# jyf588/SimGAN

Measured on AMD Instinct MI355X. Metric: env-steps/sec of GAIL-dyn PPO update, higher is better.
Workload: dtype f32; 1 GPU; northstar: GAIL-dyn update, T=128 N=512/GPU obs=47 act=12 D-in=86 policy=mlp h64 D h100 ppo_epoch=10 num_mini_batch=1...; optimizer_steps_per_update=2720, parallelism=single GPU

## Files before the change

simgan_amd/csrc/sg_disc_step4.hpp:

```cpp
#pragma once

struct Step4Args {
    PregatherArgs next;
    double* loss_acc;
};

#define SG_STEP4_TIMEOUT_TICKS 300000000ll

__device__ __forceinline__ float sg_ld_sc1(__amdgpu_buffer_rsrc_t r, int byte_off) {
    return __uint_as_float(__builtin_amdgcn_raw_buffer_load_b32(r, byte_off, 0, 16 ));
}

__device__ __forceinline__ bool sg_step4_wait(const unsigned* flags, int lo, int hi, unsigned want, int lane) {
    const long long deadline = wall_clock64() + SG_STEP4_TIMEOUT_TICKS;
    for (int it = 0;; ++it) {
        bool ok = true;
        for (int j = lo + lane; j < hi; j += 64) ok = ok & (__hip_atomic_load(flags + j * SG_STEP4_FLAG_STRIDE, __ATOMIC_RELAXED, __HIP_MEMORY_SCOPE_AGENT) == want);
        if (__all(ok)) return true;
        if ((it & 31) == 31 && wall_clock64() > deadline) return false;
        __builtin_amdgcn_s_sleep(1);
    }
}

#define SG_STEP4_POLLS 1
#define SG_STEP4_POLL_START_TICKS 340
struct SgStep4Polls { unsigned r[SG_STEP4_POLLS] = {}; };
__device__ __forceinline__ unsigned sg_step4_poll(const unsigned* p) {
    unsigned r;
    asm volatile("global_load_dword %0, %1, off sc1" : "=v"(r) : "v"(p) : "memory");
    return r;
}
__device__ __forceinline__ bool sg_step4_wait_piped(SgStep4Polls& pp, const unsigned* flags, int n, unsigned want, int lane, const int* quit) {
    constexpr int K = SG_STEP4_POLLS;
    static_assert(K >= 1 && K <= 3, "SG_STEP4_POLLS: 1, 2 or 3");
    const unsigned* p = flags + (lane < n ? lane : n - 1) * SG_STEP4_FLAG_STRIDE;
    const long long deadline = wall_clock64() + SG_STEP4_TIMEOUT_TICKS;
#pragma unroll
    for (int i = 0; i < K; ++i) {
        pp.r[i] = sg_step4_poll(p);
        if (i + 1 < K) __builtin_amdgcn_s_sleep(28 / K);
    }
    for (int it = 0;; ++it) {
#pragma unroll
        for (int i = 0; i < K; ++i) {
            asm volatile("s_waitcnt vmcnt(%1)" : "+v"(pp.r[i]) : "n"(K - 1) : "memory");
            if (__all(pp.r[i] == want)) return true;
            __builtin_amdgcn_s_sleep(1);
            pp.r[i] = sg_step4_poll(p);
        }
        if ((it & 31) == 31 && (wall_clock64() > deadline || __hip_atomic_load(quit, __ATOMIC_RELAXED, __HIP_MEMORY_SCOPE_WORKGROUP) == 2)) return false;
    }
}
__device__ __forceinline__ void sg_step4_polls_retire(SgStep4Polls& pp) {
#pragma unroll
    for (int i = 0; i < SG_STEP4_POLLS; ++i) asm volatile("" : "+v"(pp.r[i]) : : "memory");
}

template <int KF, int KH>
__global__ __launch_bounds__(512) void k_disc_step4(float* c_params, float* c_m, float* c_v, float* c_wT, float* c_ops,
                                                   SgOptState* c_st, int c_pack ,
                                                   int c_B, Step4Args a) {
    constexpr int Fp = 16 * KF, Hp = 16 * KH, ldF = Fp + 4, ldH = Hp + 4;
    constexpr int NWC = KF > KH ? KF : KH;
    constexpr int W_LDS = 8 * 256, C_LDS = SG_CHAIN4_LDS_FLOATS(KF, KH);
    __shared__ __attribute__((aligned(16))) float sm[(C_LDS > W_LDS ? C_LDS : W_LDS) + 4];
    const int c_G = c_pack & 1023, c_k1 = (int)((unsigned)c_pack >> 14);
    const int tid = threadIdx.x, wave = tid >> 6, lane = tid & 63;
    const int Kt = 64 * c_G, n_chain = 12 * c_G, w_base = (n_chain + 7) & ~7;
    unsigned* flags = reinterpret_cast<unsigned*>(c_st) + SG_STEP4_FLAG_WORD0;
    float* c_part = c_ops + (size_t)(2 - ((c_k1 - 1) & 1)) * ((size_t)Kt * (3 * Hp + ldF + Fp));

    if ((int)blockIdx.x < n_chain) {
        if (wave >= NWC) return;
        int t0 = 0;
        if (tid == 0) t0 = c_st->t0;
        Chain4Args ca{c_params, c_wT, c_ops, c_part, c_B, c_G, 1.0f / (float)c_B, 10.0f};
        sg_chain4_body<KF, KH, true>(ca, sm);
        asm volatile("s_waitcnt vmcnt(0)" ::: "memory");
        __syncthreads();
        if (tid == 0) __hip_atomic_store(flags + blockIdx.x * SG_STEP4_FLAG_STRIDE, (unsigned)(t0 + c_k1), __ATOMIC_RELAXED, __HIP_MEMORY_SCOPE_AGENT);
        return;
    }
    const int wb = (int)blockIdx.x - w_base;
    constexpr int th = KH, tf = KF, T2 = th * th, ntv = 8 * (th + tf), NV = (3 * Hp + 4 + 63) / 64;
    static_assert((8 - th) * (th + tf) > NV, "k_disc_step4: a spare slot must exist for the Adam-scalar lane");
    if (wb < 0) return;
    if (wb >= ntv) {
        if (a.next.ops) sg_disc_pregather(a.next, wb - ntv);
        return;
    }
    SgDiscDesc d;
    d.F = 0; d.Hd = 0; d.Hp = Hp; d.Fp = Fp; d.ldF = ldF; d.ldH = ldH;
    d.w1 = 0; d.b1 = Hp * ldF; d.w2 = d.b1 + Hp; d.b2 = d.w2 + Hp * ldH; d.w3 = d.b2 + Hp; d.b3 = d.w3 + Hp; d.total = d.b3 + 16;
    float (*red)[256] = reinterpret_cast<float (*)[256]>(sm);
    int* sh_ok = reinterpret_cast<int*>(sm + W_LDS);
    unsigned* err = reinterpret_cast<unsigned*>(c_st) + SG_STEP4_ERR_WORD;
    const int xcd = wb & 7, slot = wb >> 3;
    const int li = lane & 15, lq = lane >> 4;
    constexpr int nw = 8;
    if (xcd < th) {
        const int b = slot < th ? xcd * th + slot : T2 + xcd * tf + (slot - th);
        const bool w2 = b < T2;
        const int t = w2 ? b : b - T2;
        const int tm = w2 ? t / th : t / tf, tn = w2 ? t % th : t % tf;
        const int ldp = w2 ? ldH : ldF;
        const int idx = (w2 ? d.w2 : d.w1) + (tm * 16 + ((tid & 255) >> 4)) * ldp + tn * 16 + (tid & 15);
        float p0 = 0.f, m0 = 0.f, v0 = 0.f;
        float4 sc = float4{0.f, 0.f, 1.f, 1.f};
        int t0 = 0;
        if (tid < 256) {
            p0 = c_params[idx]; m0 = c_m[idx]; v0 = c_v[idx];
            sc = *reinterpret_cast<const float4*>(c_st->step_size2);
        }
        if (tid < 256 || wave >= 6) t0 = c_st->t0;
        const SgStacks stk = sg_disc_stacks(c_ops, Kt, Hp, Fp, ldF);
        const float* L = (w2 ? stk.L2 : stk.L1) + (size_t)tm * Kt * 16;
        const float* Rr = (w2 ? stk.R2 : stk.R1t) + (size_t)tn * Kt * 16;
        const int n_chunks = Kt >> 4;
        const __amdgpu_buffer_rsrc_t rL = __builtin_amdgcn_make_buffer_rsrc(const_cast<float*>(L), 0, Kt * 64, 0x00020000);
        const __amdgpu_buffer_rsrc_t rR = __builtin_amdgcn_make_buffer_rsrc(const_cast<float*>(Rr), 0, Kt * 64, 0x00020000);
        int img0 = 0, img1 = 0;
        sg_disc_img_pos(d, w2, tm * 16 + ((tid & 255) >> 4), tn * 16 + (tid & 15), img0, img1);
        const int half_chunks = n_chunks >> 1;
        auto batch_offs = [&](int c0, int c_hi, int (&o)[2][4]) {
#pragma unroll
            for (int cc = 0; cc < 2; ++cc)
#pragma unroll
                for (int s = 0; s < 4; ++s) {
                    const int c = c0 + cc * nw;
                    const int r = c < c_hi ? 16 * c + 4 * s + lq : Kt;
                    o[cc][s] = (r * 16 + li) * 4;
                }
        };
        const int mix0 = half_chunks + ((wave - half_chunks) & (nw - 1));
        int oa[2][4], ob[2][4];
        batch_offs(wave, half_chunks, oa);
        batch_offs(mix0, n_chunks, ob);
#pragma unroll
        for (int cc = 0; cc < 2; ++cc)
#pragma unroll
            for (int s = 0; s < 4; ++s) asm volatile("" : "+v"(oa[cc][s]), "+v"(ob[cc][s]));
        int* sh_bce = sh_ok + 1;
        int* sh_mix = sh_ok + 2;
        if (tid == 0) { *sh_bce = 0; *sh_mix = 0; }
        const long long poll_from = wall_clock64() + SG_STEP4_POLL_START_TICKS;
        __syncthreads();
        const unsigned want = (unsigned)(t0 + c_k1);
        auto word_set = [&](int* w, bool up) {
            if (lane == 0) __hip_atomic_store(w, up ? 1 : 2, __ATOMIC_RELAXED, __HIP_MEMORY_SCOPE_WORKGROUP);
        };
        auto word_up = [&](int* w) -> bool {
            int s;
            while ((s = __hip_atomic_load(w, __ATOMIC_RELAXED, __HIP_MEMORY_SCOPE_WORKGROUP)) == 0) __builtin_amdgcn_s_sleep(1);
            asm volatile("" ::: "memory");
            return s == 1;
        };
        SgStep4Polls pp;
        if (wave == 7) {
            word_set(sh_bce, __hip_atomic_load(err, __ATOMIC_RELAXED, __HIP_MEMORY_SCOPE_AGENT) == 0 && sg_step4_wait(flags, 4 * c_G, n_chain, want, lane));
        } else if (wave == 6) {
            bool up = __hip_atomic_load(err, __ATOMIC_RELAXED, __HIP_MEMORY_SCOPE_AGENT) == 0;
            if (up) {
                while (wall_clock64() < poll_from) __builtin_amdgcn_s_sleep(2);
                up = 4 * c_G <= 64 ? sg_step4_wait_piped(pp, flags, 4 * c_G, want, lane, sh_bce) : sg_step4_wait(flags, 0, 4 * c_G, want, lane);
            }
            word_set(sh_mix, up);
        }
        f32x4 acc = f32x4{0.f, 0.f, 0.f, 0.f}, alt = acc;
        auto load_offs = [&](const int (&o)[2][4], float (&x)[2][4], float (&y)[2][4]) {
#pragma unroll
            for (int cc = 0; cc < 2; ++cc)
#pragma unroll
                for (int s = 0; s < 4; ++s) {
                    x[cc][s] = sg_ld_sc1(rL, o[cc][s]);
                    y[cc][s] = sg_ld_sc1(rR, o[cc][s]);
                }
        };
        auto load_batch = [&](int c0, int c_hi, float (&x)[2][4], float (&y)[2][4]) {
            int o[2][4];
            batch_offs(c0, c_hi, o);
            load_offs(o, x, y);
        };
        auto mma_batch = [&](const float (&x)[2][4], const float (&y)[2][4]) {
#pragma unroll
            for (int cc = 0; cc < 2; ++cc)
#pragma unroll
                for (int s = 0; s < 4; ++s) {
                    if (s & 1) alt = sg_mfma(x[cc][s], y[cc][s], alt);
                    else acc = sg_mfma(x[cc][s], y[cc][s], acc);
                }
        };
        float xa[2][4], ya[2][4], xb[2][4], yb[2][4];
        bool up = word_up(sh_bce);
        if (up) {
            load_offs(oa, xa, ya);
            up = word_up(sh_mix);
        }
        if (!up) { if (tid == 0) { atomicOr(err, 1u); a.loss_acc[0] = __builtin_nanf(""); } return; }
        load_offs(ob, xb, yb);
        __builtin_amdgcn_sched_barrier(0);
        mma_batch(xa, ya);
        for (int c0 = wave + 2 * nw; c0 < half_chunks; c0 += 2 * nw) { load_batch(c0, half_chunks, xa, ya); mma_batch(xa, ya); }
        mma_batch(xb, yb);
        for (int c0 = mix0 + 2 * nw; c0 < n_chunks; c0 += 2 * nw) { load_batch(c0, n_chunks, xb, yb); mma_batch(xb, yb); }
        acc += alt;
#pragma unroll
        for (int r = 0; r < 4; ++r) red[wave][(4 * lq + r) * 16 + li] = acc[r];
        sg_step4_polls_retire(pp);
        __syncthreads();
        if (tid < 256) {
            float g = 0.f;
            {
                float r8[8];
#pragma unroll
                for (int w = 0; w < 8; ++w) r8[w] = red[w][tid];
#pragma unroll
                for (int w = 0; w < 8; ++w) g += r8[w];
            }
            const bool odd = (t0 + c_k1) & 1;
            const float step_size = odd ? sc.y : sc.x, bc2_sqrt = odd ? sc.w : sc.z;
            m0 = m0 + (g - m0) * (float)(1.0 - 0.9);
            v0 = v0 * (float)0.999 + (float)(1.0 - 0.999) * g * g;
            const float denom = sqrtf(v0) / bc2_sqrt + SG_DISC_ADAM_EPS;
            p0 = p0 - step_size * (m0 / denom);
            __builtin_amdgcn_sched_barrier(0);
            __builtin_nontemporal_store(p0, c_params + idx);
            __builtin_nontemporal_store(m0, c_m + idx);
            __builtin_nontemporal_store(v0, c_v + idx);
            __builtin_nontemporal_store(p0, c_wT + img0);
            __builtin_nontemporal_store(p0, c_wT + img1);
        }
        return;
    }
    const int vid = (xcd - th) * (th + tf) + slot;
    if (vid > NV) return;
    if (vid == NV) {
        if (tid == 0) sg_opt_prepare(c_st, c_st->t0 + c_k1 + 1);
        return;
    }
    {
        const int nparts = n_chain, stride = 4 * Hp, NE = 3 * Hp + 4;
        const int i = 64 * vid + lane;
        const float4 sc = *reinterpret_cast<const float4*>(c_st->step_size2);
        const int t0 = c_st->t0;
        const bool odd = (t0 + c_k1) & 1;
        const float step_size = odd ? sc.y : sc.x, bc2_sqrt = odd ? sc.w : sc.z;
        const bool is_param = wave == 0 && i < 3 * Hp + 1;
        const int pidx = i < Hp ? d.b1 + i : i < 2 * Hp ? d.b2 + (i - Hp) : i < 3 * Hp ? d.w3 + (i - 2 * Hp) : d.b3;
        float pv = 0.f, pm = 0.f, pvv = 0.f;
        if (is_param) { pv = c_params[pidx]; pm = c_m[pidx]; pvv = c_v[pidx]; }
        const __amdgpu_buffer_rsrc_t rP = __builtin_amdgcn_make_buffer_rsrc(c_part, 0, nparts * stride * 4, 0x00020000);
        if (tid == 0) *sh_ok = 1;
        __syncthreads();
        if (wave == 7 && (__hip_atomic_load(err, __ATOMIC_RELAXED, __HIP_MEMORY_SCOPE_AGENT) != 0 || !sg_step4_wait(flags, 0, n_chain, (unsigned)(t0 + c_k1), lane)) && lane == 0) *sh_ok = 0;
        __syncthreads();
        if (!*sh_ok) { if (tid == 0) { atomicOr(err, 1u); a.loss_acc[0] = __builtin_nanf(""); } return; }
        float g = 0.f;
        if (i < NE) {
            for (int s0 = wave; s0 < nparts; s0 += 16 * nw) {
                float tt[16];
#pragma unroll
                for (int u = 0; u < 16; ++u) {
                    const int sidx = s0 + u * nw;
                    tt[u] = sidx < nparts ? sg_ld_sc1(rP, (sidx * stride + i) * 4) : 0.f;
                }
#pragma unroll
                for (int u = 0; u < 16; ++u) g += tt[u];
            }
        }
        red[wave][lane] = g;
        __syncthreads();
        if (wave == 0 && i < NE) {
            g = 0.f;
            {
                float r8[8];
#pragma unroll
                for (int w = 0; w < 8; ++w) r8[w] = red[w][lane];
#pragma unroll
                for (int w = 0; w < 8; ++w) g += r8[w];
            }
            if (i < 3 * Hp + 1) {
                pm = pm + (g - pm) * (float)(1.0 - 0.9);
                pvv = pvv * (float)0.999 + (float)(1.0 - 0.999) * g * g;
                const float denom = sqrtf(pvv) / bc2_sqrt + SG_DISC_ADAM_EPS;
                c_params[pidx] = pv - step_size * (pm / denom);
                c_m[pidx] = pm;
                c_v[pidx] = pvv;
            }
            const int l0 = (3 * Hp) & 63;
            const float el_s = __shfl(g, l0 + 1), pl_s = __shfl(g, l0 + 2), gp_s = __shfl(g, l0 + 3);
            if (i == 3 * Hp) {
                const float inv_B = 1.0f / (float)c_B;
                const float el = el_s * inv_B, pl = pl_s * inv_B, gp = 10.0f * (gp_s * inv_B);
                a.loss_acc[0] += (double)(el + pl + gp);
                a.loss_acc[1] += (double)el;
                a.loss_acc[2] += (double)pl;
            }
        }
    }
}
```

Measured before the change: 2.557 million env-steps/s.

## Split reducer wait into staged flag groups and prefetch partials before readiness

The Adam-update (reducer) blocks of the discriminator step kernel no longer wait for every chain block's flag before loading partial gradients. Two waves now poll separately: one for the BCE-chain partials and one, pipelined, for the mixing/penalty partials. BCE partials are loaded as soon as their group is ready, and loss accumulators are read ahead of time. This hides part of the cross-block synchronization latency behind memory loads, at the cost of more register pressure and more complex handshake logic.

```diff
diff --git a/simgan_amd/csrc/sg_disc_step4.hpp b/simgan_amd/csrc/sg_disc_step4.hpp
--- a/simgan_amd/csrc/sg_disc_step4.hpp
+++ b/simgan_amd/csrc/sg_disc_step4.hpp
@@ -54,6 +54,16 @@
 __device__ __forceinline__ void sg_step4_polls_retire(SgStep4Polls& pp) {
 #pragma unroll
     for (int i = 0; i < SG_STEP4_POLLS; ++i) asm volatile("" : "+v"(pp.r[i]) : : "memory");
+}
+
+__device__ __forceinline__ void sg_step4_word_set(int* w, bool up, int lane) {
+    if (lane == 0) __hip_atomic_store(w, up ? 1 : 2, __ATOMIC_RELAXED, __HIP_MEMORY_SCOPE_WORKGROUP);
+}
+__device__ __forceinline__ bool sg_step4_word_up(int* w) {
+    int s;
+    while ((s = __hip_atomic_load(w, __ATOMIC_RELAXED, __HIP_MEMORY_SCOPE_WORKGROUP)) == 0) __builtin_amdgcn_s_sleep(1);
+    asm volatile("" ::: "memory");
+    return s == 1;
 }
 
 template <int KF, int KH>
@@ -146,15 +156,8 @@
         const long long poll_from = wall_clock64() + SG_STEP4_POLL_START_TICKS;
         __syncthreads();
         const unsigned want = (unsigned)(t0 + c_k1);
-        auto word_set = [&](int* w, bool up) {
-            if (lane == 0) __hip_atomic_store(w, up ? 1 : 2, __ATOMIC_RELAXED, __HIP_MEMORY_SCOPE_WORKGROUP);
-        };
-        auto word_up = [&](int* w) -> bool {
-            int s;
-            while ((s = __hip_atomic_load(w, __ATOMIC_RELAXED, __HIP_MEMORY_SCOPE_WORKGROUP)) == 0) __builtin_amdgcn_s_sleep(1);
-            asm volatile("" ::: "memory");
-            return s == 1;
-        };
+        auto word_set = [&](int* w, bool up) { sg_step4_word_set(w, up, lane); };
+        auto word_up = [&](int* w) -> bool { return sg_step4_word_up(w); };
         SgStep4Polls pp;
         if (wave == 7) {
             word_set(sh_bce, __hip_atomic_load(err, __ATOMIC_RELAXED, __HIP_MEMORY_SCOPE_AGENT) == 0 && sg_step4_wait(flags, 4 * c_G, n_chain, want, lane));
@@ -250,14 +253,54 @@
         float pv = 0.f, pm = 0.f, pvv = 0.f;
         if (is_param) { pv = c_params[pidx]; pm = c_m[pidx]; pvv = c_v[pidx]; }
         const __amdgpu_buffer_rsrc_t rP = __builtin_amdgcn_make_buffer_rsrc(c_part, 0, nparts * stride * 4, 0x00020000);
-        if (tid == 0) *sh_ok = 1;
-        __syncthreads();
-        if (wave == 7 && (__hip_atomic_load(err, __ATOMIC_RELAXED, __HIP_MEMORY_SCOPE_AGENT) != 0 || !sg_step4_wait(flags, 0, n_chain, (unsigned)(t0 + c_k1), lane)) && lane == 0) *sh_ok = 0;
-        __syncthreads();
-        if (!*sh_ok) { if (tid == 0) { atomicOr(err, 1u); a.loss_acc[0] = __builtin_nanf(""); } return; }
+        const bool loss_lane = wave == 0 && i == 3 * Hp;
+        double* const lacc = a.loss_acc;
+        double la0 = 0.0, la1 = 0.0, la2 = 0.0;
+        if (loss_lane) { la0 = lacc[0]; la1 = lacc[1]; la2 = lacc[2]; }
+        const int oob = nparts * stride * 4;
+        int ob[16], om[16];
+#pragma unroll
+        for (int u = 0; u < 16; ++u) {
+            const int sidx = wave + u * nw;
+            const int o = (sidx * stride + i) * 4;
+            const bool in = sidx < nparts && i < NE;
+            ob[u] = in && sidx >= 4 * c_G ? o : oob;
+            om[u] = in && sidx < 4 * c_G ? o : oob;
+        }
+#pragma unroll
+        for (int u = 0; u < 16; ++u) asm volatile("" : "+v"(ob[u]), "+v"(om[u]));
+        int* sh_bce = sh_ok + 1;
+        int* sh_mix = sh_ok + 2;
+        if (tid == 0) { *sh_bce = 0; *sh_mix = 0; }
+        const long long poll_from = wall_clock64() + SG_STEP4_POLL_START_TICKS;
+        __syncthreads();
+        const unsigned want = (unsigned)(t0 + c_k1);
+        SgStep4Polls pp;
+        if (wave == 7) {
+            sg_step4_word_set(sh_bce, __hip_atomic_load(err, __ATOMIC_RELAXED, __HIP_MEMORY_SCOPE_AGENT) == 0 && sg_step4_wait(flags, 4 * c_G, n_chain, want, lane), lane);
+        } else if (wave == 6) {
+            bool up = __hip_atomic_load(err, __ATOMIC_RELAXED, __HIP_MEMORY_SCOPE_AGENT) == 0;
+            if (up) {
+                while (wall_clock64() < poll_from) __builtin_amdgcn_s_sleep(2);
+                up = 4 * c_G <= 64 ? sg_step4_wait_piped(pp, flags, 4 * c_G, want, lane, sh_bce) : sg_step4_wait(flags, 0, 4 * c_G, want, lane);
+            }
+            sg_step4_word_set(sh_mix, up, lane);
+        }
+        float tb[16], tm[16];
+        bool up = sg_step4_word_up(sh_bce);
+        if (up) {
+#pragma unroll
+            for (int u = 0; u < 16; ++u) tb[u] = sg_ld_sc1(rP, ob[u]);
+            up = sg_step4_word_up(sh_mix);
+        }
+        if (!up) { if (tid == 0) { atomicOr(err, 1u); a.loss_acc[0] = __builtin_nanf(""); } return; }
+#pragma unroll
+        for (int u = 0; u < 16; ++u) tm[u] = sg_ld_sc1(rP, om[u]);
         float g = 0.f;
+#pragma unroll
+        for (int u = 0; u < 16; ++u) g += wave + u * nw < 4 * c_G ? tm[u] : tb[u];
         if (i < NE) {
-            for (int s0 = wave; s0 < nparts; s0 += 16 * nw) {
+            for (int s0 = wave + 16 * nw; s0 < nparts; s0 += 16 * nw) {
                 float tt[16];
 #pragma unroll
                 for (int u = 0; u < 16; ++u) {
@@ -269,6 +312,7 @@
             }
         }
         red[wave][lane] = g;
+        sg_step4_polls_retire(pp);
         __syncthreads();
         if (wave == 0 && i < NE) {
             g = 0.f;
@@ -292,10 +336,10 @@
             if (i == 3 * Hp) {
                 const float inv_B = 1.0f / (float)c_B;
                 const float el = el_s * inv_B, pl = pl_s * inv_B, gp = 10.0f * (gp_s * inv_B);
-                a.loss_acc[0] += (double)(el + pl + gp);
-                a.loss_acc[1] += (double)el;
-                a.loss_acc[2] += (double)pl;
-            }
-        }
-    }
-}
+                lacc[0] = la0 + (double)(el + pl + gp);
+                lacc[1] = la1 + (double)el;
+                lacc[2] = la2 + (double)pl;
+            }
+        }
+    }
+}
```

Measured after the change: 2.566 million env-steps/s (median of 6 runs). About the same (+0.4%).
